# k2-fsa/Flow2GAN

Measured on AMD Instinct MI355X. Metric: audio-seconds/sec (train step, G+D fwd/bwd) mel_24k_base, higher is better.
Workload: dtype f32 (fp32-class products on the bf16 matrix pipe for the long reductions and the direct MRD convs: every fp32 operand as three bf16 pieces = 24 significand bits, the six v_mfma_f32_32x32x16_bf16 products with i + j <= 2 per fp32 product, fp32 accumulate, error <= 2^-23 per product; short reductions ; 1 GPU; mel_24k_base GAN stage-2 train step: D-step + G-step, each on its own batch (MPD+MRD+FM+multi-scale mel), fwd+bwd+grad all-reduce, no optimizer (metric is fwd/bwd); per_gpu_batch=64, gan=gan_multi_scale_mel_recon, parallelism=dp1, optimizer=none

## Files before the change

### flow2gan_amd/_lib.py

```python
from __future__ import annotations

import ctypes as C
import os

import torch

_HERE = os.path.dirname(os.path.abspath(__file__))
LIB_PATH = os.environ.get("F2G_LIB_PATH") or os.path.join(_HERE, "libflow2gan_hip.so")

c_float_p = C.c_void_p


class Operand(C.Structure):
    _fields_ = [
        ("base", C.c_void_p), ("rows", C.c_int32), ("cols", C.c_int32),
        ("P1", C.c_int32), ("P0", C.c_int32), ("seglen", C.c_int32),
        ("step1", C.c_int32), ("pad1", C.c_int32), ("L1", C.c_int32),
        ("step0", C.c_int32), ("pad0", C.c_int32), ("unit", C.c_int32), ("L0u", C.c_int32),
        ("seq_stride", C.c_int64), ("line_stride", C.c_int64),
        ("reflect", C.c_int32), ("split", C.c_int32),
        ("alpha", C.c_void_p), ("lrelu_src", C.c_void_p),
        ("lrelu_slope", C.c_float), ("unbounded", C.c_int32),
        ("rscale", C.c_void_p),
    ]
# ... 184 lines not shown
    "f2g_conv33_wgrad": [C.POINTER(Conv32Desc), _P],
    "f2g_conv32_s2_wgrad": [C.POINTER(Conv32Desc), _P],
    "f2g_conv32_s2_wgrad_h3": [C.POINTER(Conv32Desc), _P],
    "f2g_conv2ch_fwd": [C.POINTER(Conv2chDesc)],
    "f2g_conv2ch_wgrad": [C.POINTER(Conv2chDesc)],
    "f2g_conv2ch_dgrad": [C.POINTER(Conv2chDesc)],
    "f2g_convpost_fwd": [C.POINTER(Conv2chDesc)],
    "f2g_convpost_wgrad": [C.POINTER(Conv2chDesc)],
    "f2g_convpost_dgrad": [C.POINTER(Conv2chDesc)],
    "f2g_wave_stats": [_P, _L, _L, _I, _I, _P, _P],
    "f2g_wave_gain": [_P, _L, _P, _L, _L, _I, _I, _I, _P, _P, _P],
    "f2g_sadam_stats": [_P, _P, _I, _P, _I],
    "f2g_sadam_prepare": [_P, C.POINTER(SadamGroup), _P, _P, _P, _P],
    "f2g_lrelu_bwd_colsum": [_P, _P, _P, _F, _P, _F, _I, _I, _L, _P],
    "f2g_lrelu_bwd_add": [_P, _P, _L, _I, _I, _I, _I, _L, _L, _L, _P, _L, _L, _L, _L, _F, _P],
    "f2g_zero_halo": [_P, _I, _I, _I, _I, _I],
    "f2g_sadam_update": [_P, _P, _I, _P],
    "f2g_mlp_pack": [_P, _P, _L, _P, _L, _I, _I],
    "f2g_fused_mlp": [C.POINTER(FusedMlpDesc)],
    "f2g_fused_block": [C.POINTER(DwnormFwd), C.POINTER(FusedMlpDesc)],
    "f2g_fused_block_multi": [C.POINTER(DwnormFwd), C.POINTER(FusedMlpDesc), C.c_int32],
    "f2g_istft_ola_multi": [C.POINTER(OlaMultiDesc), _P, _I, _I, _F, _I],
    "f2g_split_bf16x3": [_P, _P, _L, _I, _I],
    "f2g_split_f16x2": [_P, _P, _P, _L, _I, _I],
    "f2g_split_f16x2_cols": [_P, _P, _P, _P, _L, _I, _I],
    "f2g_split_f16x2_seq": [_P, _P, _P, _L, _I, _I],
    "f2g_multi": [C.POINTER(MultiDesc)],
}
EXPORTS = sorted(list(_SIGS) + ["f2g_version", "f2g_last_error", "f2g_gemm_last_path", "f2g_gemm_last_kernel",
                                 "f2g_fused_last_launch",
                                 "f2g_gemm_lean_ok", "f2g_gemm_wgrad_lean", "f2g_fused_mlp_ok",
                                 "f2g_dwnorm_bwd_workspace", "f2g_split_bf16x3_bytes", "f2g_gemm_x6_ok",
                                 "f2g_gemm_colsum_part_rows", "f2g_gemm_f16_ok", "f2g_set_option", "f2g_get_option",
                                 "f2g_dwconv_bwd_workspace", "f2g_sadam_chunk_elems"])


class F2GError(RuntimeError):
    pass


def _load():
    if not os.path.exists(LIB_PATH):
        raise ImportError(
            f"{LIB_PATH} is missing: build it with `python -c 'import __graft_entry__ as g; "
            "g.build()'` (or `make -C flow2gan_amd/csrc`). There is no CPU fallback.")
    lib = C.CDLL(LIB_PATH)
    for name, args in _SIGS.items():
        fn = getattr(lib, name)
        fn.argtypes = list(args) + [C.c_void_p]
        fn.restype = C.c_int
    for name in ("f2g_dwnorm_bwd_workspace", "f2g_dwconv_bwd_workspace"):
        fn = getattr(lib, name)
        fn.argtypes = [C.c_int32] * 4
        fn.restype = C.c_int64
    lib.f2g_gemm_lean_ok.argtypes = [C.POINTER(GemmDesc)]
    lib.f2g_gemm_lean_ok.restype = C.c_int
    lib.f2g_gemm_wgrad_lean.argtypes = [C.POINTER(GemmDesc)]
    lib.f2g_gemm_wgrad_lean.restype = C.c_int
    lib.f2g_split_bf16x3_bytes.argtypes = [C.c_int32, C.c_int32]
    lib.f2g_split_bf16x3_bytes.restype = C.c_int64
    lib.f2g_gemm_x6_ok.argtypes = [C.POINTER(GemmDesc)]
    lib.f2g_gemm_x6_ok.restype = C.c_int
    lib.f2g_gemm_f16_ok.argtypes = [C.POINTER(GemmDesc)]
    lib.f2g_gemm_f16_ok.restype = C.c_int
    lib.f2g_gemm_colsum_part_rows.argtypes = [C.POINTER(GemmDesc)]
    lib.f2g_gemm_colsum_part_rows.restype = C.c_int32
    lib.f2g_fused_mlp_ok.argtypes = [C.c_int32, C.c_int32]
    lib.f2g_fused_mlp_ok.restype = C.c_int
    lib.f2g_sadam_chunk_elems.argtypes = []
    lib.f2g_sadam_chunk_elems.restype = C.c_int32
    lib.f2g_set_option.argtypes = [C.c_char_p, C.c_int32]
    lib.f2g_set_option.restype = C.c_int
    lib.f2g_get_option.argtypes = [C.c_char_p, C.POINTER(C.c_int32)]
    lib.f2g_get_option.restype = C.c_int
    lib.f2g_version.restype = C.c_char_p
    lib.f2g_last_error.restype = C.c_char_p
    lib.f2g_gemm_last_kernel.argtypes = []
    lib.f2g_gemm_last_kernel.restype = C.c_char_p
    lib.f2g_fused_last_launch.argtypes = []
    lib.f2g_fused_last_launch.restype = C.c_char_p
    return lib


lib = _load()


def version() -> str:
    return lib.f2g_version().decode()


def set_option(name: str, value: int) -> int:
    old = C.c_int32()
    if lib.f2g_get_option(name.encode(), C.byref(old)) or lib.f2g_set_option(name.encode(), int(value)):
        raise F2GError(f"unknown library option {name!r}")
    return old.value


def get_option(name: str) -> int:
    v = C.c_int32()
    if lib.f2g_get_option(name.encode(), C.byref(v)):
        raise F2GError(f"unknown library option {name!r}")
    return v.value


def has_option(name: str) -> bool:
    return lib.f2g_get_option(name.encode(), C.byref(C.c_int32())) == 0


def stream_ptr() -> int:
    return torch.cuda.current_stream().cuda_stream


def ptr(t) -> int | None:
    if t is None:
        return None
    if not t.is_cuda:
        raise F2GError("flow2gan_amd ops need tensors on an MI355X (got a CPU tensor)")
    if t.dtype not in (torch.float32, torch.int32, torch.bfloat16):
        raise F2GError(f"unsupported dtype {t.dtype}")
    return t.data_ptr()


_DRYRUN = os.environ.get("F2G_DRYRUN", "0") == "1"


PRE_CALL = None


def call(name: str, *args):
    if PRE_CALL is not None and name != "f2g_multi":
        PRE_CALL()
    if _DRYRUN:
        stream_ptr()
        return
    rc = getattr(lib, name)(*args, stream_ptr())
# ... 3 lines not shown
```

### flow2gan_amd/csrc/capi.hip

```cpp
#include <stdio.h>
#include <stdlib.h>
#include <string.h>
#include <strings.h>

#include <mutex>

#include "common.h"
#include "version_gen.h"

static char g_err[256] = "";

void f2g_set_error(const char* msg) {
  strncpy(g_err, msg ? msg : "", sizeof(g_err) - 1);
  g_err[sizeof(g_err) - 1] = 0;
}

int f2g_check_launch() {
  hipError_t e = hipGetLastError();
  if (e != hipSuccess) {
    f2g_set_error(hipGetErrorString(e));
    return F2G_ELAUNCH;
  }
  return F2G_OK;
}

extern "C" const char* f2g_version(void) { return "flow2gan_hip 0.4.0 src:" F2G_SRC_HASH " gfx950"; }
extern "C" const char* f2g_last_error(void) { return g_err; }

namespace {
struct Opt { const char* name; int value; };
Opt g_opts[F2G_OPT_COUNT] = {
    {"lean_tall", 1}, {"lean_wgrad", 1}, {"x6p", 1}, {"deterministic", 0}, {"streamk", 1}, {"mlp_rt", 0},
    {"mlp_split", 0}, {"multi_rt384", 4}, {"multi_rt512", 3}, {"streamk_min", 4}};
std::once_flag g_opts_once;

int opt_index(const char* name, size_t len) {
  for (int i = 0; i < F2G_OPT_COUNT; ++i)
    if (strlen(g_opts[i].name) == len && strncasecmp(g_opts[i].name, name, len) == 0) return i;
  return -1;
}

void opts_init() {
  const char* e = getenv("F2G_OPTS");
  while (e && *e) {
    const char* end = strchr(e, ',');
    const size_t len = end ? (size_t)(end - e) : strlen(e);
    const char* eq = (const char*)memchr(e, '=', len);
    if (eq) {
      const int i = opt_index(e, (size_t)(eq - e));
      if (i >= 0) g_opts[i].value = atoi(eq + 1);
    }
    e = end ? end + 1 : nullptr;
  }
  const char* det = getenv("F2G_DETERMINISTIC");
  if (det) g_opts[F2G_OPT_DETERMINISTIC].value = atoi(det) != 0;
}
}

int f2g_opt(int id) {
  std::call_once(g_opts_once, opts_init);
  return g_opts[id].value;
}

extern "C" int f2g_set_option(const char* name, int32_t value) {
  std::call_once(g_opts_once, opts_init);
  const int i = name ? opt_index(name, strlen(name)) : -1;
// ... 16 lines not shown
```

### flow2gan_amd/csrc/common.h

```cpp
#pragma once
#include <hip/hip_runtime.h>
#include <stdint.h>

#include <type_traits>

#include "../../include/flow2gan_hip.h"

int f2g_check_launch();
void f2g_note_kernel(const char* name, int split, int path);
enum f2g_opt_id {
  F2G_OPT_LEAN_TALL,
  F2G_OPT_LEAN_WGRAD,
  F2G_OPT_X6P,
  F2G_OPT_DETERMINISTIC,
  F2G_OPT_STREAMK,
  F2G_OPT_MLP_RT,
  F2G_OPT_MLP_SPLIT,
  F2G_OPT_MULTI_RT384,
  F2G_OPT_MULTI_RT512,
  F2G_OPT_STREAMK_MIN,
  F2G_OPT_COUNT
};
int f2g_opt(int id);
int f2g_gemm_narrow(const f2g_gemm_desc& d, hipStream_t st);
void f2g_set_error(const char* msg);
int f2g_x6p_ok(const f2g_gemm_desc& d, int taps);
int f2g_launch_x6p(const f2g_gemm_desc& d, int taps, long long a_extent, hipStream_t st);
int f2g_leanw6t_ok(const f2g_gemm_desc& d, int split);
int f2g_launch_leanw6t(const f2g_gemm_desc& d, int split, hipStream_t st);
struct f2g_colsegs {
  float* out[3];
  int begin[3];
  int count[3];
};
int f2g_colsum_segments(const float* a, long long lda, int rows, int ncols,
                        const f2g_colsegs& segs, hipStream_t st);

#define F2G_WAVE 64

__device__ __forceinline__ float wave_sum(float v) {
#pragma unroll
  for (int o = 32; o > 0; o >>= 1) v += __shfl_xor(v, o);
  return v;
}

__device__ __forceinline__ float wave_max(float v) {
#pragma unroll
  for (int o = 32; o > 0; o >>= 1) v = fmaxf(v, __shfl_xor(v, o));
  return v;
}

typedef float f2g_f32x2 __attribute__((ext_vector_type(2)));
typedef __bf16 f2g_bf16x2 __attribute__((ext_vector_type(2)));
// ... 26 lines not shown
```

### flow2gan_amd/csrc/conv32_common.h

```cpp
#pragma once
#include "common.h"

namespace {

typedef float f32x16 __attribute__((ext_vector_type(16)));
typedef float f32x4 __attribute__((ext_vector_type(4)));
typedef __bf16 bf16x8 __attribute__((ext_vector_type(8)));
typedef unsigned int u32x2 __attribute__((ext_vector_type(2)));
typedef short s16x4 __attribute__((ext_vector_type(4)));

constexpr int C = 32;
constexpr int KH = 3, KW = 9;

__device__ __attribute__((aligned(16))) float c32_zero[4] = {0.f, 0.f, 0.f, 0.f};

__device__ __forceinline__ constexpr int acc_row(int e) { return (e & 3) + 8 * (e >> 2); }

__device__ __forceinline__ bf16x8 tr_pix8(const unsigned char* p) {
  typedef s16x4 __attribute__((address_space(3))) * lds_p;
  const s16x4 a = __builtin_amdgcn_ds_read_tr16_b64_v4i16((lds_p)(p));
  const s16x4 b = __builtin_amdgcn_ds_read_tr16_b64_v4i16((lds_p)(p + 4 * 64));
  return __builtin_bit_cast(bf16x8, __builtin_shufflevector(a, b, 0, 1, 2, 3, 4, 5, 6, 7));
}

template <int D>
__device__ __forceinline__ int div_small(int x) {
  static_assert(D == 39 || D == 23 || D == 20 || D == 12, "magic constants below");
  return (x * (D == 39 ? 1681 : D == 23 ? 2850 : D == 20 ? 3277 : 5462)) >> 16;
}

template <int TW_>
__device__ __forceinline__ void px_of_row(int pg, int r, int& ph, int& pw) {
  if (TW_ == 16) {
    ph = 2 * pg + (r >> 4);
    pw = (r + 12 * (r >> 4)) & 15;
  } else {
    const int p = pg * 32 + r;
    ph = p / TW_;
    pw = p % TW_;
  }
}

struct c32_tiling {
  bool tall;
  int tiles_h, tiles_w, tiles_w_also;
};
inline c32_tiling c32_pick_tiles(int H, int W, int W_also = 0) {
  auto waste = [&](int th, int tw) {
    return (long long)((H + th - 1) / th * th) * ((W + tw - 1) / tw * tw + (W_also + tw - 1) / tw * tw);
  };
  const bool tall = waste(16, 8) < waste(8, 16);
  const int th = tall ? 16 : 8, tw = tall ? 8 : 16;
  return {tall, (H + th - 1) / th, (W + tw - 1) / tw, (W_also + tw - 1) / tw};
}

template <auto KERNEL>
inline void c32_lds_once(size_t smem) {
  static const hipError_t done = [&] {
    return hipFuncSetAttribute(reinterpret_cast<const void*>(KERNEL), hipFuncAttributeMaxDynamicSharedMemorySize,
                               (int)smem);
  }();
  (void)done;
}

template <auto K8x16, auto K16x8, typename... Args>
inline int c32_launch_shape(bool tall, size_t smem8x16, size_t smem16x8, dim3 grid, dim3 block, hipStream_t st,
                            Args... args) {
  c32_lds_once<K8x16>(smem8x16);
  c32_lds_once<K16x8>(smem16x8);
  if (tall) hipLaunchKernelGGL(K16x8, grid, block, smem16x8, st, args...);
  else hipLaunchKernelGGL(K8x16, grid, block, smem8x16, st, args...);
  return f2g_check_launch();
}

template <typename REF>
__device__ __forceinline__ float c32_mask_fm(float v, float y, bool fm, REF ref, float fmw, float mask_slope) {
  if (fm) {
    const float dl = y - ref();
    v += fmw * (dl > 0.f ? 1.f : (dl < 0.f ? -1.f : 0.f));
  }
  return v * (y > 0.f ? 1.f : mask_slope);
}

template <int NT, int OWN>
__device__ __forceinline__ void c32_wgrad_flush(float* gw, float* red_, const f32x16 (&acc)[OWN + NT - 8 * OWN],
                                                int wave, int lane, int li, int hh) {
  typedef float __attribute__((address_space(3))) * lds_f;
  const lds_f red = (lds_f)red_;
#pragma unroll
  for (int q = 0; q < OWN; ++q) {
    const int t = wave + 8 * q;
#pragma unroll
    for (int e = 0; e < 16; ++e) atomicAdd(gw + (acc_row(e) + 4 * hh) * (NT * C) + t * C + li, acc[q][e]);
  }
#pragma unroll
  for (int q = 0; q < NT - 8 * OWN; ++q) {
    __syncthreads();
#pragma unroll
    for (int e = 0; e < 16; ++e) red[(wave * 16 + e) * 64 + lane] = acc[OWN + q][e];
    __syncthreads();
    if (wave == (q & 7)) {
#pragma unroll
      for (int e = 0; e < 16; ++e) {
        float v = 0.f;
// ... 10 lines not shown
```

### flow2gan_amd/csrc/conv32x6.hip

```cpp
#include <stdlib.h>

#include "conv32_common.h"

namespace {

typedef unsigned int u32x4 __attribute__((ext_vector_type(4)));

constexpr int NTAP = KH * KW;
constexpr int PB = 208;

__device__ __forceinline__ void split3(const f32x4 v, u32x2& p0, u32x2& p1, u32x2& p2) {
  unsigned a0, a1, a2, b0, b1, b2;
  f2g_split3_pair(v.x, v.y, a0, a1, a2);
  f2g_split3_pair(v.z, v.w, b0, b1, b2);
  p0 = u32x2{a0, b0};
  p1 = u32x2{a1, b1};
  p2 = u32x2{a2, b2};
}

__device__ __forceinline__ void store_px3(unsigned char* p, const f32x4 v) {
  u32x2 p0, p1, p2;
  split3(v, p0, p1, p2);
  *reinterpret_cast<u32x2*>(p) = p0;
  *reinterpret_cast<u32x2*>(p + 64) = p1;
// ... 145 lines not shown
    __syncthreads();
#pragma unroll
    for (int p2 = 0; p2 < 2; ++p2) {
      if (p2) __syncthreads();
#pragma unroll
      for (int g2 = 0; g2 < 2; ++g2)
#pragma unroll
        for (int e = 0; e < 16; ++e)
          red[((wave * 2 + g2) * 32 + acc_row(e) + 4 * hh) * 32 + li] = acc[2 * p2 + g2][e];
      __syncthreads();
      f32x4 s = *reinterpret_cast<const f32x4*>(red + (((wave >> 2)) * 32 + orow) * 32 + och);
#pragma unroll
      for (int w8 = 1; w8 < 8; ++w8) {
        const f32x4 v = *reinterpret_cast<const f32x4*>(red + ((w8 * 2 + (wave >> 2)) * 32 + orow) * 32 + och);
        s.x += v.x, s.y += v.y, s.z += v.z, s.w += v.w;
      }
      s.x += bias4.x, s.y += bias4.y, s.z += bias4.z, s.w += bias4.w;
      if (d.lrelu_slope != 0.f) {
        s.x = s.x > 0.f ? s.x : d.lrelu_slope * s.x;
        s.y = s.y > 0.f ? s.y : d.lrelu_slope * s.y;
        s.z = s.z > 0.f ? s.z : d.lrelu_slope * s.z;
        s.w = s.w > 0.f ? s.w : d.lrelu_slope * s.w;
      }
      int qh, qw;
      px_of_row<TW_>(2 * p2 + (wave >> 2), orow, qh, qw);
      const int oh = h0 + qh, ow = w0 + qw;
      if (oh < d.H && ow < d.Wout)
        *reinterpret_cast<f32x4*>(ys + (long long)oh * d.y_line + (long long)ow * C + och) = s;
      if (p2 == 0 && more) store_patch(pf);
    }
  }
}

template <int TH_, int TW_>
__global__ __launch_bounds__(512, 1) void conv32_s2_dgrad6_kernel(const f2g_conv32_desc d, int tiles_w,
                                                                 int tiles_h, int ntiles) {
  constexpr int IHv = TH_ + KH - 1, GWv = TW_ + 4;
  constexpr int NCHK = (IHv * GWv * (C / 4) + 511) / 512;
  constexpr int PGB = (TW_ == 16 ? 2 : 4) * GWv * PB;
  constexpr int KPW = 8;
  static_assert(TH_ * TW_ == 128, "a block owns 128 positions of each column parity");
  extern __shared__ __attribute__((aligned(16))) unsigned char smb[];
  unsigned char* At = smb;
  float* red = reinterpret_cast<float*>(smb + IHv * GWv * PB);
  const int tid = threadIdx.x, lane = tid & 63;
  const int wave = __builtin_amdgcn_readfirstlane(tid >> 6);
  const int li = lane & 31, hh = lane >> 5;
  const int wq = wave & 3, E = wave >> 2;
  const int c4 = tid & 7;
  const int NU = E ? 4 : 5;
  const int Wp = (d.Win + 1 - E) / 2;
  const int px0 = tid >> 3;
  auto tile_pos = [&](int tile, int& sq, int& h0, int& m0) {
    const int tw = tile % tiles_w, rest = tile / tiles_w;
    const int th = rest % tiles_h;
    sq = rest / tiles_h;
    h0 = th * TH_;
    m0 = tw * TW_;
  };
  auto load_patch = [&](int tile, f32x4 (&pf)[NCHK]) {
    int sq, h0, m0;
    tile_pos(tile, sq, h0, m0);
    const float* org = d.x + (long long)sq * d.x_seq + (long long)(h0 - 1) * d.x_line + (long long)(m0 - 2) * C + c4 * 4;
    const int xl = (int)d.x_line;
    int pxb = px0;
    asm volatile("" : "+v"(pxb));
#pragma unroll
    for (int q = 0; q < NCHK; ++q) {
      const int px = pxb + 64 * q;
      const int r = div_small<GWv>(px), xc = px - r * GWv;
      const int h = h0 - 1 + r, c = m0 - 2 + xc;
      const bool ok = px < IHv * GWv && h >= 0 && h < d.H && c >= 0 && c < d.Wout;
      pf[q] = *reinterpret_cast<const f32x4*>(ok ? org + (r * xl + xc * C) : c32_zero);
    }
  };
  auto store_patch = [&](const f32x4 (&pf)[NCHK]) {
#pragma unroll
    for (int q = 0; q < NCHK; ++q) {
      const int px = px0 + 64 * q;
      if (px < IHv * GWv) store_px3(At + px * PB + c4 * 8, pf[q]);
    }
  };
  int tile = blockIdx.x;
  if (tile >= ntiles) return;
  f32x4 pf[NCHK];
  load_patch(tile, pf);
  const int nk = E ? 6 : (wq < 2 ? 8 : 7);
  const int k0 = E ? 6 * wq : (wq < 2 ? 8 * wq : 16 + 7 * (wq - 2));
  bf16x8 wf[KPW][3];
  int koff[KPW];
  {
    const unsigned char* wrow = reinterpret_cast<const unsigned char*>(d.w) + li * 192 + hh * 16;
    const int nks = 2 * KH * NU;
#pragma unroll
    for (int j = 0; j < KPW; ++j) {
      int k = k0 + j;
      k = k < nks ? k : nks - 1;
      const int ti = k >> 1, ks = k & 1;
      const int dh = E ? ti >> 2 : (ti * 13) >> 6;
      const int u = ti - dh * NU;
      koff[j] = ks * 32 - (dh * GWv + u) * PB;
      const int tile_w = dh * KW + E + 2 * u;
#pragma unroll
      for (int q = 0; q < 3; ++q)
        wf[j][q] = *reinterpret_cast<const bf16x8*>(wrow + tile_w * (C * 192) + q * 64 + ks * 32);
    }
  }
  int ph, pw;
  px_of_row<TW_>(0, li, ph, pw);
  const unsigned char* Ap = At + ((ph + 2) * GWv + pw + 4) * PB + hh * 16;
  const int och = 4 * (lane & 7);
  const bool msk = d.mask_src != nullptr, fm = d.fm_ref != nullptr;
  const float fmw = fm ? d.fm_w * (d.fm_wdev ? d.fm_wdev[0] : 1.f) : 0.f;
  float cs[4] = {0.f, 0.f, 0.f, 0.f};
  store_patch(pf);
  __syncthreads();
  for (; tile < ntiles; tile += gridDim.x) {
    const int nxt = tile + gridDim.x;
    const bool more = nxt < ntiles;
    load_patch(more ? nxt : tile, pf);
    int sq, h0, m0;
    tile_pos(tile, sq, h0, m0);
    const long long tbase = (long long)sq * d.y_seq + (long long)h0 * d.y_line + (long long)(2 * m0 + E) * C;
    auto item_off = [&](int jj) {
      int qh, qw, l8 = lane >> 3;
      asm volatile("" : "+v"(l8));
      px_of_row<TW_>(2 * (jj >> 1) + (wq >> 1), (wq & 1) * 16 + l8 + 8 * (jj & 1), qh, qw);
      return (h0 + qh < d.H && m0 + qw < Wp) ? qh * (int)d.y_line + 2 * qw * C + och : -1;
    };
    f32x4 my[4];
    if (msk && !fm) {
#pragma unroll
      for (int jj = 0; jj < 4; ++jj) {
        const int o = item_off(jj);
        my[jj] = *reinterpret_cast<const f32x4*>(d.mask_src + (o >= 0 ? tbase + o : 0));
      }
    }
    f32x16 acc[4];
#pragma unroll
    for (int g4 = 0; g4 < 4; ++g4)
#pragma unroll
      for (int e = 0; e < 16; ++e) acc[g4][e] = 0.f;
    bf16x8 a[2][3];
// ... 70 lines not shown
      v += __shfl_xor(v, 8);
      v += __shfl_xor(v, 16);
      v += __shfl_xor(v, 32);
      if (lane < 8) csl[wave * 32 + 4 * lane + e] = v;
    }
    __syncthreads();
    if (tid < 32) {
      float v = csl[tid];
#pragma unroll
      for (int w8 = 1; w8 < 8; ++w8) v += csl[w8 * 32 + tid];
      atomicAdd(d.colsum + tid, v);
    }
  }
}

constexpr int GPL = 128 * 64;
constexpr int GCH = 128 * (C / 4) / 512;

template <int TH, int TW>
constexpr size_t wgrad6_smem() {
  return (size_t)3 * 2 * ((TH + KH - 1) * (TW + (KW - 1) / 2) * 64 + 64) + 3 * GPL;
}

template <int TH, int TW>
__global__ __launch_bounds__(512, 1) void conv32_s2_wgrad6_kernel(const f2g_conv32_desc d, float* gw,
                                                                  int tiles_h, int tiles_w,
                                                                  int tiles_per_block) {
  constexpr int IH = TH + KH - 1, IW = TW + (KW - 1) / 2, XW = 2 * IW - 1;
  constexpr int XPAR = IH * IW * 64 + 64;
  constexpr int XPL = 2 * XPAR;
  constexpr int XCH = (IH * XW * (C / 4) + 511) / 512;
  constexpr int KR = 16 / TW;
  constexpr int NK = TH / KR;
  static_assert(TH * TW == 128 && NK == 8 && XCH <= NK && GCH <= NK, "tile shapes");
  extern __shared__ __attribute__((aligned(16))) unsigned char smb[];
  unsigned char* Xp = smb;
  unsigned char* Gp = smb + 3 * XPL;
  const int tid = threadIdx.x, lane = tid & 63, wave = tid >> 6;
  const int li = lane & 31, hh = lane >> 5;
  const int ntiles = d.S * tiles_h * tiles_w;
  f32x16 acc[6];
#pragma unroll
  for (int a = 0; a < 6; ++a)
#pragma unroll
    for (int e = 0; e < 16; ++e) acc[a][e] = 0.f;
  const int g4 = lane >> 4, i16 = lane & 15;
  const int kpix = (g4 >> 1) * 8 + (i16 >> 2);
  const int kpat = TW == 16 ? kpix : (g4 >> 1) * IW + (i16 >> 2);
  const int chb = (g4 & 1) * 32 + (i16 & 3) * 8;
  int xo[3], xs[3];
#pragma unroll
  for (int a = 0; a < 3; ++a) {
    int t = wave + 8 * a;
    int dh = t / KW, j = t - dh * KW;
    xo[a] = (j & 1) * XPAR + (dh * IW + (j >> 1) + kpat) * 64 + chb;
    t = 24 + a;
    dh = t / KW;
    j = t - dh * KW;
    xs[a] = (j & 1) * XPAR + (dh * IW + (j >> 1) + kpat) * 64 + chb;
  }
  const int go = kpix * 64 + chb;
  const int c4 = tid & 7, px0 = tid >> 3;
  auto xoff = [&](int q) {
    const int px = px0 + 64 * q;
    const int r = div_small<XW>(px), xr = px - r * XW;
    return px < IH * XW ? (xr & 1) * XPAR + (r * IW + (xr >> 1)) * 64 + c4 * 8 : -1;
  };
  auto tile_pos = [&](int ti, int& s, int& h0, int& w0) {
    s = ti / (tiles_h * tiles_w);
    const int rem = ti - s * (tiles_h * tiles_w);
    const int th = rem / tiles_w;
    h0 = th * TH;
    w0 = (rem - th * tiles_w) * TW;
  };
  auto load_tile = [&](int ti, f32x4 (&px_)[XCH], f32x4 (&pg_)[GCH]) {
    int s, h0, w0;
    tile_pos(ti, s, h0, w0);
    const int x0 = 2 * w0 - (KW - 1) / 2;
    const float* org = d.x + (long long)s * d.x_seq + (long long)(h0 - 1) * d.x_line + (long long)x0 * C + c4 * 4;
#pragma unroll
    for (int q = 0; q < XCH; ++q) {
// ... 28 lines not shown
  }
  {
    f32x4 px_[XCH], pg_[GCH];
    load_tile(t0, px_, pg_);
#pragma unroll
    for (int q = 0; q < XCH; ++q)
      if (xoff(q) >= 0) {
        u32x2 pk[3];
        split3(px_[q], pk[0], pk[1], pk[2]);
        put3(Xp, XPL, xoff(q), pk);
      }
#pragma unroll
    for (int q = 0; q < GCH; ++q) {
      u32x2 pk[3];
      split3(pg_[q], pk[0], pk[1], pk[2]);
      put3(Gp, GPL, ((tid >> 3) + 64 * q) * 64 + c4 * 8, pk);
    }
  }
  __syncthreads();
  for (int ti = t0; ti < tend; ++ti) {
    const bool more = ti + 1 < tend;
    f32x4 px_[XCH], pg_[GCH];
    u32x2 kx[XCH][3], kg[GCH][3];
    load_tile(more ? ti + 1 : ti, px_, pg_);
#pragma unroll
    for (int row = 0; row < NK; ++row) {
      bf16x8 a[3];
#pragma unroll
      for (int q = 0; q < 3; ++q) a[q] = tr_pix8(Gp + q * GPL + go + row * 16 * 64);
#pragma unroll
      for (int t = 0; t < 3; ++t) {
        bf16x8 b[3];
#pragma unroll
        for (int q = 0; q < 3; ++q) b[q] = tr_pix8(Xp + q * XPL + xo[t] + row * KR * IW * 64);
        mfma6(a, b, acc[t]);
      }
      if (row < XCH) split3(px_[row < XCH ? row : 0], kx[row < XCH ? row : 0][0], kx[row < XCH ? row : 0][1], kx[row < XCH ? row : 0][2]);
      if (row >= NK - GCH)
        split3(pg_[row >= NK - GCH ? row - (NK - GCH) : 0], kg[row >= NK - GCH ? row - (NK - GCH) : 0][0],
               kg[row >= NK - GCH ? row - (NK - GCH) : 0][1], kg[row >= NK - GCH ? row - (NK - GCH) : 0][2]);
    }
    {
      const int row = wave;
      bf16x8 a[3];
#pragma unroll
      for (int q = 0; q < 3; ++q) a[q] = tr_pix8(Gp + q * GPL + go + row * 16 * 64);
#pragma unroll
      for (int t = 0; t < 3; ++t) {
        bf16x8 b[3];
#pragma unroll
        for (int q = 0; q < 3; ++q) b[q] = tr_pix8(Xp + q * XPL + xs[t] + row * KR * IW * 64);
        mfma6(a, b, acc[3 + t]);
      }
    }
    __syncthreads();
    if (more) {
#pragma unroll
      for (int q = 0; q < XCH; ++q)
        if (xoff(q) >= 0) put3(Xp, XPL, xoff(q), kx[q]);
#pragma unroll
      for (int q = 0; q < GCH; ++q) put3(Gp, GPL, ((tid >> 3) + 64 * q) * 64 + c4 * 8, kg[q]);
    }
    __syncthreads();
  }
  static_assert(wgrad6_smem<TH, TW>() >= (size_t)8 * 16 * 64 * 4, "the flush reuses the planes as its reduction buffer");
  c32_wgrad_flush<NTAP, 3>(gw, reinterpret_cast<float*>(smb), acc, wave, lane, li, hh);
}

constexpr int P33 = 352;
constexpr int T33 = 9;

__global__ __launch_bounds__(512, 1) void conv33_x6_kernel(const f2g_conv32_desc d, int R, int tiles_h, int ntiles) {
  extern __shared__ __attribute__((aligned(16))) unsigned char smb[];
  unsigned char* At = smb;
  unsigned char* Bt = smb + P33 * PB;
  const int tid = threadIdx.x, lane = tid & 63, wave = tid >> 6;
  const int li = lane & 31, hh = lane >> 5;
  const int W = d.Win, PW = W + 2, npx = (R + 2) * PW, tpx = R * W;
  const unsigned mgW = magic_of(W), mgPW = magic_of(PW);
  {
    const unsigned char* wimg = reinterpret_cast<const unsigned char*>(d.w);
    for (int c = tid; c < T33 * C * 12; c += 512) {
      const int row = c / 12, part = c - row * 12;
      const int co = row / T33, tap = row - co * T33;
// ... 154 lines not shown
#pragma unroll
        for (int pc = 0; pc < 3; ++pc) *reinterpret_cast<u32x2*>(Xp + pc * W33_XPL + (px + 1) * 64 + c4 * 8) = pk[pc];
      }
      if (grow[q] > -(1 << 21)) {
        split3(pg_[q], pk[0], pk[1], pk[2]);
#pragma unroll
        for (int pc = 0; pc < 3; ++pc) *reinterpret_cast<u32x2*>(Gp + pc * W33_GPL + px * 64 + c4 * 8) = pk[pc];
      }
    }
    __syncthreads();
    for (int ks = wave; ks < nks; ks += 8) {
      bf16x8 a[3];
#pragma unroll
      for (int q = 0; q < 3; ++q) a[q] = tr_pix8(Gp + q * W33_GPL + ks * (16 * 64) + go);
#pragma unroll
      for (int t = 0; t < T33; ++t) {
        bf16x8 b[3];
#pragma unroll
        for (int q = 0; q < 3; ++q) b[q] = tr_pix8(Xp + q * W33_XPL + ks * (16 * 64) + xo[t]);
        mfma6(a, b, acc[t]);
      }
    }
    __syncthreads();
  }
  c32_wgrad_flush<T33, 0>(gw, reinterpret_cast<float*>(smb), acc, wave, lane, li, hh);
}

template <int TH_, int TW_>
constexpr size_t fwd6_smem() {
  return (size_t)2 * ((TH_ + 2) * (TW_ + 4) * PB + 64) + 8 * 2 * 32 * 32 * sizeof(float);
}
template <int TH_, int TW_>
constexpr size_t dgrad6_smem() {
  return (size_t)(TH_ + 2) * (TW_ + 4) * PB + 8 * 2 * 32 * 32 * sizeof(float);
}

}

int f2g_conv32_fwd6_launch(const f2g_conv32_desc* d, hipStream_t st) {
  const c32_tiling t = c32_pick_tiles(d->H, d->Wout);
  const long long nt = (long long)t.tiles_h * t.tiles_w * d->S;
  if (nt >= (1ll << 30) || d->x_line >= (1ll << 24)) return F2G_EINVAL;
  const int grid = (int)(nt < 256 ? nt : 256);
  return c32_launch_shape<conv32_s2_fwd6_kernel<8, 16>, conv32_s2_fwd6_kernel<16, 8>>(
      t.tall, fwd6_smem<8, 16>(), fwd6_smem<16, 8>(), dim3(grid), dim3(512), st, *d, t.tiles_w, t.tiles_h, (int)nt);
}

int f2g_conv32_dgrad6_launch(const f2g_conv32_desc* d, hipStream_t st) {
  const c32_tiling t = c32_pick_tiles(d->H, (d->Win + 1) / 2);
  const long long nt = (long long)t.tiles_h * t.tiles_w * d->S;
  if (nt >= (1ll << 30) || d->x_line >= (1ll << 24) || d->y_line >= (1ll << 24)) return F2G_EINVAL;
  const int grid = (int)(nt < 256 ? nt : 256);
  return c32_launch_shape<conv32_s2_dgrad6_kernel<8, 16>, conv32_s2_dgrad6_kernel<16, 8>>(
      t.tall, dgrad6_smem<8, 16>(), dgrad6_smem<16, 8>(), dim3(grid), dim3(512), st, *d, t.tiles_w, t.tiles_h,
      (int)nt);
}

int f2g_conv32_wgrad6_launch(const f2g_conv32_desc* d, float* gw, hipStream_t st) {
  const c32_tiling t = c32_pick_tiles(d->H, d->Wout);
  const long long nt = (long long)d->S * t.tiles_h * t.tiles_w;
  if (nt >= (1ll << 30) || d->x_line >= (1ll << 24)) return F2G_EINVAL;
  int per = (int)((nt + 255) / 256);
  if (per < 1) per = 1;
  const unsigned grid = (unsigned)((nt + per - 1) / per);
  return c32_launch_shape<conv32_s2_wgrad6_kernel<8, 16>, conv32_s2_wgrad6_kernel<16, 8>>(
      t.tall, wgrad6_smem<8, 16>(), wgrad6_smem<16, 8>(), dim3(grid), dim3(512), st, *d, gw, t.tiles_h, t.tiles_w,
      per);
}

extern "C" int f2g_conv33_fwd(const f2g_conv32_desc* d, f2g_stream_t stream) {
  if (!d || !d->x || !d->w || !d->y || d->precision != 3 || d->Win != d->Wout || d->fm_ref) return F2G_EINVAL;
  if ((((uintptr_t)d->x) & 15) || (((uintptr_t)d->w) & 15) || (d->x_line & 3) || (d->x_seq & 3)) return F2G_EINVAL;
  if (d->S <= 0 || d->H <= 0 || d->Win <= 0) return F2G_OK;
  const int W = d->Win;
  if (W > 112 || d->x_line >= (1ll << 24)) return F2G_EINVAL;
  if (d->y_line < (long long)W * C || (d->y != d->x && d->y_seq < (long long)d->H * d->y_line)) return F2G_EINVAL;
  if ((d->y_line & 3) || (d->y_seq & 3) || (((uintptr_t)d->y) & 15)) return F2G_EINVAL;
  if (d->mask_src && (d->lrelu_slope != 0.f || d->bias || (((uintptr_t)d->mask_src) & 15))) {
    f2g_set_error("f2g_conv33_fwd: mask_src (data-gradient role) excludes bias / lrelu_slope (forward role)");
    return F2G_EINVAL;
  }
  int R = 256 / W;
  if (R > d->H) R = d->H;
  while (R > 1 && (R + 2) * (W + 2) > P33) --R;
  if (R < 1 || (R + 2) * (W + 2) > P33) return F2G_EINVAL;
  const int tiles_h = (d->H + R - 1) / R;
  const long long nt = (long long)tiles_h * d->S;
  if (nt >= (1ll << 30)) return F2G_EINVAL;
  constexpr size_t smem = (size_t)P33 * PB + (size_t)T33 * C * PB;
  c32_lds_once<conv33_x6_kernel>(smem);
  const int grid = (int)(nt < 256 ? nt : 256);
  hipLaunchKernelGGL(conv33_x6_kernel, dim3(grid), dim3(512), smem, (hipStream_t)stream, *d, R, tiles_h, (int)nt);
  return f2g_check_launch();
}

extern "C" int f2g_conv33_wgrad(const f2g_conv32_desc* d, float* gw, f2g_stream_t stream) {
  if (!d || !d->x || !d->y || !gw || d->precision != 3 || d->Win != d->Wout) return F2G_EINVAL;
  if ((((uintptr_t)d->x) & 15) || (((uintptr_t)d->y) & 15) || (d->x_line & 3) || (d->x_seq & 3) || (d->y_line & 3) ||
      (d->y_seq & 3))
    return F2G_EINVAL;
// ... 22 lines not shown
```

### include/flow2gan_hip.h

```cpp
#ifndef FLOW2GAN_HIP_H
#define FLOW2GAN_HIP_H

#include <stdint.h>

#ifdef __cplusplus
extern "C" {
#endif

typedef void* f2g_stream_t;

enum {
  F2G_OK = 0,
  F2G_EINVAL = -1,
  F2G_ELAUNCH = -2,
};

const char* f2g_version(void);
const char* f2g_last_error(void);

int f2g_set_option(const char* name, int32_t value);
int f2g_get_option(const char* name, int32_t* value);

typedef struct {
  const float* base;
// ... 278 lines not shown
  const float* g;
  const float* mask_src;
  const float* fm_ref;
  const float* fm_wdev;
  float mask_slope;
  float fm_w;
  float* colsum;
  void* x3_out;
} f2g_mpdpost_desc;
int f2g_mpdpost_fwd(const f2g_mpdpost_desc* d, f2g_stream_t stream);
int f2g_mpdpost_dgrad(const f2g_mpdpost_desc* d, f2g_stream_t stream);
int f2g_mpdpost_wgrad(const f2g_mpdpost_desc* d, float* gw, f2g_stream_t stream);

typedef struct {
  const float* x;
  int64_t x_seq, x_line;
  int32_t S, H, Win, Wout;
  const float* w;
  const float* bias;
  float lrelu_slope;
  int32_t precision;
  float* y;
  int64_t y_seq, y_line;
  const float* mask_src;
  const float* fm_ref;
  const float* fm_wdev;
  float mask_slope;
  float fm_w;
  float* colsum;
} f2g_conv32_desc;
int f2g_conv32_s2_fwd(const f2g_conv32_desc* d, f2g_stream_t stream);
int f2g_conv32_s2_dgrad(const f2g_conv32_desc* d, f2g_stream_t stream);
int f2g_conv32_s2_wgrad(const f2g_conv32_desc* d, float* gw, f2g_stream_t stream);
int f2g_conv32_s2_wgrad_h3(const f2g_conv32_desc* d, float* gw, f2g_stream_t stream);
int f2g_conv33_fwd(const f2g_conv32_desc* d, f2g_stream_t stream);
int f2g_conv33_wgrad(const f2g_conv32_desc* d, float* gw, f2g_stream_t stream);

typedef struct {
  const float* x;
  int64_t x_seq, x_line;
  int32_t S, H, W, _pad;
  const float* w;
  const float* bias;
  float lrelu_slope;
  int32_t _pad2;
  float* y;
  float* gw;
  const float* wt;
  float* gx;
  int64_t gx_seq, gx_line;
} f2g_conv2ch_desc;
int f2g_conv2ch_fwd(const f2g_conv2ch_desc* d, f2g_stream_t stream);
int f2g_conv2ch_wgrad(const f2g_conv2ch_desc* d, f2g_stream_t stream);
int f2g_conv2ch_dgrad(const f2g_conv2ch_desc* d, f2g_stream_t stream);
int f2g_convpost_fwd(const f2g_conv2ch_desc* d, f2g_stream_t stream);
int f2g_convpost_wgrad(const f2g_conv2ch_desc* d, f2g_stream_t stream);
int f2g_convpost_dgrad(const f2g_conv2ch_desc* d, f2g_stream_t stream);

int f2g_wave_stats(const float* x, int64_t item_stride, int64_t ch_stride, int32_t B, int32_t C,
                   const int32_t* lens, float* stats, f2g_stream_t stream);
int f2g_wave_gain(float* out, int64_t ldo, const float* x, int64_t item_stride, int64_t ch_stride,
                  int32_t B, int32_t C, int32_t T, const int32_t* lens, const float* stats,
                  const float* target_peak, f2g_stream_t stream);

#define F2G_SADAM_NCOEF 12
#define F2G_SADAM_TSTATE 10
// ... 61 lines not shown
```

Baseline: 817.0 audio-s/s.

## Add 32x4 tile shape for conv32 dgrad/wgrad kernels with waste-based selection

Adds a narrow 32x4 tile variant for the stride-2 data-gradient and weight-gradient MFMA conv kernels. A generalized picker chooses among 16/8/4-wide tiles by padded-area waste, so narrow MRD spectrogram widths pad less. The dgrad LDS pitch and the wgrad transposed-read offsets are adjusted for the new width, and an option plus a query API can force a specific shape. The risk is that narrow tiles use LDS or read patterns less efficiently, or that tile selection flips on shapes where 4-wide is worse.

New measurement: 819.4 audio-s/s, median of 6. Within noise of the previous version (+0.3%).

```diff
diff --git a/flow2gan_amd/_lib.py b/flow2gan_amd/_lib.py
--- a/flow2gan_amd/_lib.py
+++ b/flow2gan_amd/_lib.py
@@ -240,7 +240,7 @@
                                  "f2g_gemm_lean_ok", "f2g_gemm_wgrad_lean", "f2g_fused_mlp_ok",
                                  "f2g_dwnorm_bwd_workspace", "f2g_split_bf16x3_bytes", "f2g_gemm_x6_ok",
                                  "f2g_gemm_colsum_part_rows", "f2g_gemm_f16_ok", "f2g_set_option", "f2g_get_option",
-                                 "f2g_dwconv_bwd_workspace", "f2g_sadam_chunk_elems"])
+                                 "f2g_dwconv_bwd_workspace", "f2g_sadam_chunk_elems", "f2g_conv32_tile_shape"])
 
 
 class F2GError(RuntimeError):
@@ -281,6 +281,8 @@
     lib.f2g_set_option.restype = C.c_int
     lib.f2g_get_option.argtypes = [C.c_char_p, C.POINTER(C.c_int32)]
     lib.f2g_get_option.restype = C.c_int
+    lib.f2g_conv32_tile_shape.argtypes = [C.c_int32] * 4 + [C.POINTER(C.c_int32)] * 2
+    lib.f2g_conv32_tile_shape.restype = C.c_int
     lib.f2g_version.restype = C.c_char_p
     lib.f2g_last_error.restype = C.c_char_p
     lib.f2g_gemm_last_kernel.argtypes = []
@@ -309,6 +311,13 @@
     if lib.f2g_get_option(name.encode(), C.byref(v)):
         raise F2GError(f"unknown library option {name!r}")
     return v.value
+
+
+def conv32_tile_shape(role: int, H: int, Win: int, Wout: int):
+    th, tw = C.c_int32(), C.c_int32()
+    if lib.f2g_conv32_tile_shape(role, H, Win, Wout, C.byref(th), C.byref(tw)):
+        raise F2GError("f2g_conv32_tile_shape refused its arguments")
+    return th.value, tw.value
 
 
 def has_option(name: str) -> bool:
diff --git a/flow2gan_amd/csrc/capi.hip b/flow2gan_amd/csrc/capi.hip
--- a/flow2gan_amd/csrc/capi.hip
+++ b/flow2gan_amd/csrc/capi.hip
@@ -31,7 +31,8 @@
 struct Opt { const char* name; int value; };
 Opt g_opts[F2G_OPT_COUNT] = {
     {"lean_tall", 1}, {"lean_wgrad", 1}, {"x6p", 1}, {"deterministic", 0}, {"streamk", 1}, {"mlp_rt", 0},
-    {"mlp_split", 0}, {"multi_rt384", 4}, {"multi_rt512", 3}, {"streamk_min", 4}};
+    {"mlp_split", 0}, {"multi_rt384", 4}, {"multi_rt512", 3}, {"streamk_min", 4},
+    {"conv32_tile", 0}};
 std::once_flag g_opts_once;
 
 int opt_index(const char* name, size_t len) {
diff --git a/flow2gan_amd/csrc/common.h b/flow2gan_amd/csrc/common.h
--- a/flow2gan_amd/csrc/common.h
+++ b/flow2gan_amd/csrc/common.h
@@ -19,6 +19,7 @@
   F2G_OPT_MULTI_RT384,
   F2G_OPT_MULTI_RT512,
   F2G_OPT_STREAMK_MIN,
+  F2G_OPT_CONV32_TILE,
   F2G_OPT_COUNT
 };
 int f2g_opt(int id);
diff --git a/flow2gan_amd/csrc/conv32_common.h b/flow2gan_amd/csrc/conv32_common.h
--- a/flow2gan_amd/csrc/conv32_common.h
+++ b/flow2gan_amd/csrc/conv32_common.h
@@ -1,5 +1,6 @@
 #pragma once
 #include "common.h"
+#include "conv32_tiles.h"
 
 namespace {
 
@@ -16,17 +17,23 @@
 
 __device__ __forceinline__ constexpr int acc_row(int e) { return (e & 3) + 8 * (e >> 2); }
 
+template <int SECOND = 4 * 64>
 __device__ __forceinline__ bf16x8 tr_pix8(const unsigned char* p) {
   typedef s16x4 __attribute__((address_space(3))) * lds_p;
   const s16x4 a = __builtin_amdgcn_ds_read_tr16_b64_v4i16((lds_p)(p));
-  const s16x4 b = __builtin_amdgcn_ds_read_tr16_b64_v4i16((lds_p)(p + 4 * 64));
+  const s16x4 b = __builtin_amdgcn_ds_read_tr16_b64_v4i16((lds_p)(p + SECOND));
   return __builtin_bit_cast(bf16x8, __builtin_shufflevector(a, b, 0, 1, 2, 3, 4, 5, 6, 7));
 }
 
+constexpr bool div_small_exact(int D) {
+  for (int x = 0; x < 512; ++x)
+    if (((x * ((65536 + D - 1) / D)) >> 16) != x / D) return false;
+  return true;
+}
 template <int D>
 __device__ __forceinline__ int div_small(int x) {
-  static_assert(D == 39 || D == 23 || D == 20 || D == 12, "magic constants below");
-  return (x * (D == 39 ? 1681 : D == 23 ? 2850 : D == 20 ? 3277 : 5462)) >> 16;
+  static_assert(D >= 2 && D <= 64 && div_small_exact(D), "the multiply-shift below is exact for x < 512");
+  return (x * ((65536 + D - 1) / D)) >> 16;
 }
 
 template <int TW_>
@@ -39,19 +46,6 @@
     ph = p / TW_;
     pw = p % TW_;
   }
-}
-
-struct c32_tiling {
-  bool tall;
-  int tiles_h, tiles_w, tiles_w_also;
-};
-inline c32_tiling c32_pick_tiles(int H, int W, int W_also = 0) {
-  auto waste = [&](int th, int tw) {
-    return (long long)((H + th - 1) / th * th) * ((W + tw - 1) / tw * tw + (W_also + tw - 1) / tw * tw);
-  };
-  const bool tall = waste(16, 8) < waste(8, 16);
-  const int th = tall ? 16 : 8, tw = tall ? 8 : 16;
-  return {tall, (H + th - 1) / th, (W + tw - 1) / tw, (W_also + tw - 1) / tw};
 }
 
 template <auto KERNEL>
@@ -70,6 +64,13 @@
   c32_lds_once<K16x8>(smem16x8);
   if (tall) hipLaunchKernelGGL(K16x8, grid, block, smem16x8, st, args...);
   else hipLaunchKernelGGL(K8x16, grid, block, smem8x16, st, args...);
+  return f2g_check_launch();
+}
+
+template <auto KERNEL, typename... Args>
+inline int c32_launch_one(size_t smem, dim3 grid, dim3 block, hipStream_t st, Args... args) {
+  c32_lds_once<KERNEL>(smem);
+  hipLaunchKernelGGL(KERNEL, grid, block, smem, st, args...);
   return f2g_check_launch();
 }
 
diff --git a/flow2gan_amd/csrc/conv32_tiles.h b/flow2gan_amd/csrc/conv32_tiles.h
--- /dev/null
+++ b/flow2gan_amd/csrc/conv32_tiles.h
@@ -0,0 +1,20 @@
+#pragma once
+
+constexpr unsigned C32_WIDE = 16 | 8;
+
+struct c32_tiling {
+  bool tall;
+  int th, tw;
+  int tiles_h, tiles_w, tiles_w_also;
+};
+
+inline c32_tiling c32_pick_tiles(int H, int W, int W_also = 0, unsigned widths = C32_WIDE) {
+  auto up = [](int n, int t) { return (n + t - 1) / t * t; };
+  auto padded = [&](int tw) { return (long long)up(H, 128 / tw) * (up(W, tw) + up(W_also, tw)); };
+  int tw = 0;
+  for (int c = 16; c >= 2; c >>= 1)
+    if ((widths & c) && (!tw || padded(c) < padded(tw))) tw = c;
+  if (!tw) tw = 16;
+  const int th = 128 / tw;
+  return {tw == 8, th, tw, (H + th - 1) / th, (W + tw - 1) / tw, (W_also + tw - 1) / tw};
+}
diff --git a/flow2gan_amd/csrc/conv32x6.hip b/flow2gan_amd/csrc/conv32x6.hip
--- a/flow2gan_amd/csrc/conv32x6.hip
+++ b/flow2gan_amd/csrc/conv32x6.hip
@@ -201,17 +201,23 @@
   }
 }
 
+template <int TW_>
+constexpr int dgrad6_pitch() {
+  return TW_ == 4 ? 12 : TW_ + 4;
+}
 template <int TH_, int TW_>
 __global__ __launch_bounds__(512, 1) void conv32_s2_dgrad6_kernel(const f2g_conv32_desc d, int tiles_w,
                                                                  int tiles_h, int ntiles) {
   constexpr int IHv = TH_ + KH - 1, GWv = TW_ + 4;
+  constexpr int GP = dgrad6_pitch<TW_>();
   constexpr int NCHK = (IHv * GWv * (C / 4) + 511) / 512;
-  constexpr int PGB = (TW_ == 16 ? 2 : 4) * GWv * PB;
+  constexpr int PGB = (32 / TW_) * GP * PB;
   constexpr int KPW = 8;
-  static_assert(TH_ * TW_ == 128, "a block owns 128 positions of each column parity");
+  static_assert(TH_ * TW_ == 128 && 32 % TW_ == 0 && TW_ <= 16,
+                "a block owns 128 positions of each column parity; a position group is whole tile rows");
   extern __shared__ __attribute__((aligned(16))) unsigned char smb[];
   unsigned char* At = smb;
-  float* red = reinterpret_cast<float*>(smb + IHv * GWv * PB);
+  float* red = reinterpret_cast<float*>(smb + IHv * GP * PB);
   const int tid = threadIdx.x, lane = tid & 63;
   const int wave = __builtin_amdgcn_readfirstlane(tid >> 6);
   const int li = lane & 31, hh = lane >> 5;
@@ -247,7 +253,11 @@
 #pragma unroll
     for (int q = 0; q < NCHK; ++q) {
       const int px = px0 + 64 * q;
-      if (px < IHv * GWv) store_px3(At + px * PB + c4 * 8, pf[q]);
+      if (GP == GWv) {
+        if (px < IHv * GWv) store_px3(At + px * PB + c4 * 8, pf[q]);
+      } else {
+        if (px < IHv * GWv) store_px3(At + (px + div_small<GWv>(px) * (GP - GWv)) * PB + c4 * 8, pf[q]);
+      }
     }
   };
   int tile = blockIdx.x;
@@ -268,7 +278,7 @@
       const int ti = k >> 1, ks = k & 1;
       const int dh = E ? ti >> 2 : (ti * 13) >> 6;
       const int u = ti - dh * NU;
-      koff[j] = ks * 32 - (dh * GWv + u) * PB;
+      koff[j] = ks * 32 - (dh * GP + u) * PB;
       const int tile_w = dh * KW + E + 2 * u;
 #pragma unroll
       for (int q = 0; q < 3; ++q)
@@ -277,7 +287,7 @@
   }
   int ph, pw;
   px_of_row<TW_>(0, li, ph, pw);
-  const unsigned char* Ap = At + ((ph + 2) * GWv + pw + 4) * PB + hh * 16;
+  const unsigned char* Ap = At + ((ph + 2) * GP + pw + 4) * PB + hh * 16;
   const int och = 4 * (lane & 7);
   const bool msk = d.mask_src != nullptr, fm = d.fm_ref != nullptr;
   const float fmw = fm ? d.fm_w * (d.fm_wdev ? d.fm_wdev[0] : 1.f) : 0.f;
@@ -414,7 +424,8 @@
   constexpr int XCH = (IH * XW * (C / 4) + 511) / 512;
   constexpr int KR = 16 / TW;
   constexpr int NK = TH / KR;
-  static_assert(TH * TW == 128 && NK == 8 && XCH <= NK && GCH <= NK, "tile shapes");
+  constexpr int SEC = TW >= 8 ? 4 * 64 : IW * 64;
+  static_assert(TH * TW == 128 && TW >= 4 && NK == 8 && XCH <= NK && GCH <= NK, "tile shapes");
   extern __shared__ __attribute__((aligned(16))) unsigned char smb[];
   unsigned char* Xp = smb;
   unsigned char* Gp = smb + 3 * XPL;
@@ -428,7 +439,7 @@
     for (int e = 0; e < 16; ++e) acc[a][e] = 0.f;
   const int g4 = lane >> 4, i16 = lane & 15;
   const int kpix = (g4 >> 1) * 8 + (i16 >> 2);
-  const int kpat = TW == 16 ? kpix : (g4 >> 1) * IW + (i16 >> 2);
+  const int kpat = TW == 16 ? kpix : (g4 >> 1) * (8 / TW) * IW + (i16 >> 2);
   const int chb = (g4 & 1) * 32 + (i16 & 3) * 8;
   int xo[3], xs[3];
 #pragma unroll
@@ -523,7 +534,7 @@
       for (int t = 0; t < 3; ++t) {
         bf16x8 b[3];
 #pragma unroll
-        for (int q = 0; q < 3; ++q) b[q] = tr_pix8(Xp + q * XPL + xo[t] + row * KR * IW * 64);
+        for (int q = 0; q < 3; ++q) b[q] = tr_pix8<SEC>(Xp + q * XPL + xo[t] + row * KR * IW * 64);
         mfma6(a, b, acc[t]);
       }
       if (row < XCH) split3(px_[row < XCH ? row : 0], kx[row < XCH ? row : 0][0], kx[row < XCH ? row : 0][1], kx[row < XCH ? row : 0][2]);
@@ -540,7 +551,7 @@
       for (int t = 0; t < 3; ++t) {
         bf16x8 b[3];
 #pragma unroll
-        for (int q = 0; q < 3; ++q) b[q] = tr_pix8(Xp + q * XPL + xs[t] + row * KR * IW * 64);
+        for (int q = 0; q < 3; ++q) b[q] = tr_pix8<SEC>(Xp + q * XPL + xs[t] + row * KR * IW * 64);
         mfma6(a, b, acc[3 + t]);
       }
     }
@@ -761,13 +772,48 @@
 }
 template <int TH_, int TW_>
 constexpr size_t dgrad6_smem() {
-  return (size_t)(TH_ + 2) * (TW_ + 4) * PB + 8 * 2 * 32 * 32 * sizeof(float);
-}
-
+  return (size_t)(TH_ + 2) * dgrad6_pitch<TW_>() * PB + 8 * 2 * 32 * 32 * sizeof(float);
+}
+constexpr size_t LDS_CU = 160 * 1024;
+static_assert(fwd6_smem<32, 4>() > LDS_CU, "32 x 4 forward tiles stage 34 x 15 pixels: over 170 KB with the partial sums");
+static_assert(dgrad6_smem<32, 4>() <= LDS_CU, "32 x 4 data-gradient tiles fit");
+static_assert(wgrad6_smem<32, 4>() <= LDS_CU, "32 x 4 weight-gradient tiles fit");
+
+}
+
+namespace {
+constexpr unsigned FWD6_BUILT = C32_WIDE, DGRAD6_BUILT = C32_WIDE | 4, WGRAD6_BUILT = C32_WIDE | 4;
+constexpr unsigned FWD6_SHAPES = C32_WIDE;
+constexpr unsigned DGRAD6_SHAPES = C32_WIDE | 4;
+constexpr unsigned DGRAD6M_SHAPES = C32_WIDE | 4;
+constexpr unsigned WGRAD6_SHAPES = C32_WIDE | 4;
+
+inline unsigned shapes_of(unsigned built, unsigned dflt) {
+  const int f = f2g_opt(F2G_OPT_CONV32_TILE);
+  if (f < 0) return C32_WIDE;
+  return (f == 16 || f == 8 || f == 4) && (built & (unsigned)f) ? (unsigned)f : dflt;
+}
+
+inline c32_tiling tiling6(int role, int H, int Win, int Wout) {
+  switch (role) {
+    case 1: return c32_pick_tiles(H, (Win + 1) / 2, 0, shapes_of(DGRAD6_BUILT, DGRAD6_SHAPES));
+    case 2: return c32_pick_tiles(H, (Win + 1) / 2, 0, shapes_of(DGRAD6_BUILT, DGRAD6M_SHAPES));
+    case 3: return c32_pick_tiles(H, Wout, 0, shapes_of(WGRAD6_BUILT, WGRAD6_SHAPES));
+    default: return c32_pick_tiles(H, Wout, 0, shapes_of(FWD6_BUILT, FWD6_SHAPES));
+  }
+}
+}
+
+extern "C" int f2g_conv32_tile_shape(int32_t role, int32_t H, int32_t Win, int32_t Wout, int32_t* th, int32_t* tw) {
+  if (role < 0 || role > 3 || H <= 0 || Win <= 0 || Wout <= 0 || !th || !tw) return F2G_EINVAL;
+  const c32_tiling t = tiling6(role, H, Win, Wout);
+  *th = t.th;
+  *tw = t.tw;
+  return F2G_OK;
 }
 
 int f2g_conv32_fwd6_launch(const f2g_conv32_desc* d, hipStream_t st) {
-  const c32_tiling t = c32_pick_tiles(d->H, d->Wout);
+  const c32_tiling t = tiling6(0, d->H, d->Win, d->Wout);
   const long long nt = (long long)t.tiles_h * t.tiles_w * d->S;
   if (nt >= (1ll << 30) || d->x_line >= (1ll << 24)) return F2G_EINVAL;
   const int grid = (int)(nt < 256 ? nt : 256);
@@ -776,25 +822,37 @@
 }
 
 int f2g_conv32_dgrad6_launch(const f2g_conv32_desc* d, hipStream_t st) {
-  const c32_tiling t = c32_pick_tiles(d->H, (d->Win + 1) / 2);
+  const c32_tiling t = tiling6(d->mask_src ? 2 : 1, d->H, d->Win, d->Wout);
   const long long nt = (long long)t.tiles_h * t.tiles_w * d->S;
   if (nt >= (1ll << 30) || d->x_line >= (1ll << 24) || d->y_line >= (1ll << 24)) return F2G_EINVAL;
-  const int grid = (int)(nt < 256 ? nt : 256);
-  return c32_launch_shape<conv32_s2_dgrad6_kernel<8, 16>, conv32_s2_dgrad6_kernel<16, 8>>(
-      t.tall, dgrad6_smem<8, 16>(), dgrad6_smem<16, 8>(), dim3(grid), dim3(512), st, *d, t.tiles_w, t.tiles_h,
-      (int)nt);
+  const dim3 grid((unsigned)(nt < 256 ? nt : 256)), block(512);
+  switch (t.tw) {
+#define F2G_DGRAD6(TH_, TW_)                                                                                       \
+  case TW_:                                                                                                        \
+    return c32_launch_one<conv32_s2_dgrad6_kernel<TH_, TW_>>(dgrad6_smem<TH_, TW_>(), grid, block, st, *d, t.tiles_w, \
+                                                             t.tiles_h, (int)nt);
+    F2G_DGRAD6(8, 16) F2G_DGRAD6(16, 8) F2G_DGRAD6(32, 4)
+#undef F2G_DGRAD6
+  }
+  return F2G_EINVAL;
 }
 
 int f2g_conv32_wgrad6_launch(const f2g_conv32_desc* d, float* gw, hipStream_t st) {
-  const c32_tiling t = c32_pick_tiles(d->H, d->Wout);
+  const c32_tiling t = tiling6(3, d->H, d->Win, d->Wout);
   const long long nt = (long long)d->S * t.tiles_h * t.tiles_w;
   if (nt >= (1ll << 30) || d->x_line >= (1ll << 24)) return F2G_EINVAL;
   int per = (int)((nt + 255) / 256);
   if (per < 1) per = 1;
-  const unsigned grid = (unsigned)((nt + per - 1) / per);
-  return c32_launch_shape<conv32_s2_wgrad6_kernel<8, 16>, conv32_s2_wgrad6_kernel<16, 8>>(
-      t.tall, wgrad6_smem<8, 16>(), wgrad6_smem<16, 8>(), dim3(grid), dim3(512), st, *d, gw, t.tiles_h, t.tiles_w,
-      per);
+  const dim3 grid((unsigned)((nt + per - 1) / per)), block(512);
+  switch (t.tw) {
+#define F2G_WGRAD6(TH_, TW_)                                                                                       \
+  case TW_:                                                                                                        \
+    return c32_launch_one<conv32_s2_wgrad6_kernel<TH_, TW_>>(wgrad6_smem<TH_, TW_>(), grid, block, st, *d, gw,        \
+                                                             t.tiles_h, t.tiles_w, per);
+    F2G_WGRAD6(8, 16) F2G_WGRAD6(16, 8) F2G_WGRAD6(32, 4)
+#undef F2G_WGRAD6
+  }
+  return F2G_EINVAL;
 }
 
 extern "C" int f2g_conv33_fwd(const f2g_conv32_desc* d, f2g_stream_t stream) {
diff --git a/include/flow2gan_hip.h b/include/flow2gan_hip.h
--- a/include/flow2gan_hip.h
+++ b/include/flow2gan_hip.h
@@ -334,6 +334,7 @@
 int f2g_conv32_s2_fwd(const f2g_conv32_desc* d, f2g_stream_t stream);
 int f2g_conv32_s2_dgrad(const f2g_conv32_desc* d, f2g_stream_t stream);
 int f2g_conv32_s2_wgrad(const f2g_conv32_desc* d, float* gw, f2g_stream_t stream);
+int f2g_conv32_tile_shape(int32_t role, int32_t H, int32_t Win, int32_t Wout, int32_t* th, int32_t* tw);
 int f2g_conv32_s2_wgrad_h3(const f2g_conv32_desc* d, float* gw, f2g_stream_t stream);
 int f2g_conv33_fwd(const f2g_conv32_desc* d, f2g_stream_t stream);
 int f2g_conv33_wgrad(const f2g_conv32_desc* d, float* gw, f2g_stream_t stream);
```
